# kristi700/ViT-SSL

Hardware: AMD Instinct MI355X
Metric: images_per_sec (higher is better)
Workload: dtype bf16; 1 GPU; ViT-B/16 SimMIM 224x224 mask 0.6 dropout 0.1 AdamW, batch 256/GPU; global_batch=256, parallelism=dp1

## Files before the change

### include/vitssl_hip.h

```cpp
#ifndef VITSSL_HIP_H
#define VITSSL_HIP_H

#include <stdint.h>

#ifdef __cplusplus
extern "C" {
#endif

#define VITSSL_OK 0
#define VITSSL_ERR_ARG (-1)
#define VITSSL_ERR_LAUNCH (-2)

const char* vitssl_last_error(void);
int vitssl_version(void);

int vitssl_set_reserved_cus(int n);
int vitssl_get_reserved_cus(void);
int vitssl_debug_last_nt_grid(void);
int vitssl_debug_last_attn_fwd_grid(void);

typedef struct {
  float p;
  uint32_t site;
  uint64_t seed;
// ... 89 lines not shown
int vitssl_gemm_bf16_tn(const void* A, const void* B, float* C, int64_t M, int N1, int N2, float* workspace,
                        int64_t workspace_floats, void* stream);

typedef struct {
  const void* A;
  const void* B;
  float* C;
  int N1, N2;
} vitssl_tn_job_t;
int64_t vitssl_gemm_tn_batch_workspace_floats(const vitssl_tn_job_t* jobs, int njobs, int64_t M);
int vitssl_gemm_bf16_tn_batch(const vitssl_tn_job_t* jobs, int njobs, int64_t M, float* workspace, int64_t workspace_floats,
                              void* stream);

typedef struct {
  const void* A8;
  const void* B8;
  float* C;
  int N1, N2;
  const float* alpha;
  const float* alpha2;
} vitssl_fp8_tn_job_t;
int64_t vitssl_gemm_fp8_tn_batch_workspace_floats(const vitssl_fp8_tn_job_t* jobs, int njobs, int64_t M);
int vitssl_gemm_fp8_tn_batch(const vitssl_fp8_tn_job_t* jobs, int njobs, int64_t M, float* workspace, int64_t workspace_floats,
                             void* stream);

int vitssl_attn_fwd(const void* qkv, void* out, float* lse, float* probs, int B, int N, int H, int dh,
                    void* stream);
int vitssl_attn_bwd(const void* qkv, const void* out, const void* dout, const float* lse, void* dqkv,
                    float* delta_ws, int B, int N, int H, int dh, void* stream);

int vitssl_patchify_bf16(const float* img, void* patches, int B, int C, int H, int W, int P, void* stream);
int vitssl_gather_patches_f32(const float* img, const int32_t* idx, float* out, int n_idx, int C, int H,
                              int W, int P, void* stream);
int vitssl_gather_rows_bf16(const float* x, const int32_t* idx, void* out, int n_idx, int cols, void* stream);
int vitssl_scatter_rows_f32(const void* src_bf16, const int32_t* inv, float* g, int64_t rows, int cols,
                            void* stream);
int vitssl_gather_cls_f32(const float* x, float* out, int B, int T, int D, void* stream);
int vitssl_scatter_cls_f32(const float* gcls, float* g, int B, int T, int D, void* stream);

int64_t vitssl_embed_bwd_workspace_floats(int B, int tokens, int tok_offset, int D);
int vitssl_embed_bwd(const float* dtok, const uint8_t* mask, void* dproj_bf16, float* dpos, float* dmask_token,
                     float* dbias, float* dcls, int B, int tokens, int tok_offset, int D, float* workspace,
                     int64_t workspace_floats, void* stream);

int vitssl_l1_loss(const float* pred, const float* target, float* loss_sum, void* dpred_bf16, float gscale,
                   int64_t n, float* workspace, int64_t workspace_floats, void* stream);
int vitssl_cross_entropy(const float* logits, const int64_t* labels, float* loss_sum, void* dlogits_bf16,
                         float gscale, int B, int C, void* stream);

int vitssl_colsum_bf16(const void* x_bf16, float* out, int64_t rows, int cols, float* workspace, int64_t workspace_floats,
                       void* stream);

int64_t vitssl_sum_workspace_floats(int64_t rows, int cols);

int vitssl_cast_bf16(const float* src, void* dst, int64_t n, void* stream);
int vitssl_cast_transpose_bf16(const float* src, void* dst, void* dst_t, int R, int C, void* stream);
typedef struct {
  const float* src;
  void* dst;
  void* dst_t;
  int R, C;
} vitssl_cast_job_t;
int vitssl_cast_transpose_batch(const vitssl_cast_job_t* jobs, const int* tile_start, int njobs, int total_tiles,
                                void* stream);
int vitssl_adamw(float* p, const float* g, float* m, float* v, int64_t n, float lr, float beta1, float beta2,
                 float eps, float wd, int step, float gscale, void* stream);
int vitssl_ema(float* teacher, const float* student, int64_t n, float m, void* stream);

int vitssl_rownorm_fwd(const float* z, void* zn_bf16, float* inv_norm, int64_t rows, int cols, void* stream);
int vitssl_rownorm_bwd(const float* dzn, const void* zn_bf16, const float* inv_norm, void* dz_bf16, int64_t rows, int cols,
                       void* stream);
int vitssl_weightnorm_fold(const float* g, const float* v, float* w_f32, float* inv_vnorm, int K, int D, void* stream);
int vitssl_weightnorm_bwd(const float* dw, const float* g, const float* v, const float* inv_vnorm, float* dg, float* dv, int K,
                          int D, void* stream);
#define VITSSL_DINO_TWS_EXTRA(G, B) (8 * (G) * (B))
int64_t vitssl_dino_loss_workspace_floats(int G, int B, int K);
int vitssl_dino_loss(const float* teacher, const float* student, const float* center, float* t_ws, int64_t t_ws_floats,
                     float* loss_sum, void* dstudent_bf16, int G, int V, int B, int K, float teacher_temp, float student_temp,
                     float gscale, void* stream);
int vitssl_colsum_f32(const float* x, float* out, int64_t rows, int cols, void* stream);
int vitssl_center_ema(float* center, const float* colsum, int K, float momentum, float inv_rows, void* stream);

int vitssl_bicubic_resize_fwd(const float* src, float* dst, int gh0, int gw0, int gh, int gw, int D, void* stream);
int vitssl_bicubic_resize_bwd(const float* ddst, float* dsrc, int gh0, int gw0, int gh, int gw, int D, void* stream);

int vitssl_aug_resized_crop_u8(const uint8_t* src, const int32_t* iparams, uint8_t* tmp, uint8_t* dst, int B, int H,
                               int W, int S, void* stream);
int vitssl_aug_color_u8(uint8_t* img, const int32_t* iparams, const float* fparams, int B, int S, void* stream);
int vitssl_aug_blur_to_tensor(const uint8_t* img, const float* fparams, float* out, int B, int S, int ksize,
                              void* stream);

#ifdef __cplusplus
}
#endif
#endif
```

### vit-ssl_amd/csrc/elementwise.hip

```cpp
#include "common.h"

namespace {

constexpr int EW_THREADS = 256;

inline unsigned ew_grid(long long work_items) {
  long long g = (work_items + EW_THREADS - 1) / EW_THREADS;
  if (g < 1) g = 1;
  return (unsigned)g;
}

__global__ void dropout_mask_kernel(unsigned char* keep, long long ngroups, DropKey dk) {
  const long long grp = (long long)blockIdx.x * blockDim.x + threadIdx.x;
  if (grp >= ngroups) return;
  float m[4];
  drop_mult4(dk, (unsigned)grp, m);
  uchar4 o;
  o.x = m[0] != 0.f; o.y = m[1] != 0.f; o.z = m[2] != 0.f; o.w = m[3] != 0.f;
  if (dk.thr == 0) o = make_uchar4(1, 1, 1, 1);
  *(uchar4*)(keep + 4 * grp) = o;
}

template <bool GATHER, typename OutT>
__global__ void patchify_kernel(const float* __restrict__ img, const int* __restrict__ idx, OutT* __restrict__ out,
                                long long nrows, int C, int H, int W, int P) {
  const int gw = W / P, gh = H / P;
  const int pd4 = C * P * P / 4;
  const long long t = (long long)blockIdx.x * blockDim.x + threadIdx.x;
  if (t >= nrows * pd4) return;
  const long long r = t / pd4;
  const int f = (int)(t - r * pd4) * 4;
  const long long m = GATHER ? (long long)idx[r] : r;
  const long long b = m / (gh * gw);
  const int pi = (int)(m - b * gh * gw);
  const int py = pi / gw, px = pi - py * gw;
  const int c = f / (P * P);
  const int kh = (f - c * P * P) / P;
  const int kw = f - c * P * P - kh * P;
  const f32x4 v = *(const f32x4*)(img + ((b * C + c) * H + (py * P + kh)) * (long long)W + px * P + kw);
  if constexpr (sizeof(OutT) == 2) {
    u32x2 w = {pack_bf2(v[0], v[1]), pack_bf2(v[2], v[3])};
    *(u32x2*)((bf16_t*)out + r * (4LL * pd4) + f) = w;
  } else {
    *(f32x4*)((float*)out + r * (4LL * pd4) + f) = v;
  }
}

__global__ void gather_rows_bf16_kernel(const float* __restrict__ x, const int* __restrict__ idx, bf16_t* __restrict__ out,
                                        int n_idx, int cols) {
  const int c4n = cols >> 2;
  const long long t = (long long)blockIdx.x * blockDim.x + threadIdx.x;
  if (t >= (long long)n_idx * c4n) return;
  const int i = (int)(t / c4n);
  const int c = (int)(t - (long long)i * c4n) * 4;
  const f32x4 v = *(const f32x4*)(x + (long long)idx[i] * cols + c);
  u32x2 w = {pack_bf2(v[0], v[1]), pack_bf2(v[2], v[3])};
  *(u32x2*)(out + (long long)i * cols + c) = w;
}

__global__ void scatter_rows_f32_kernel(const bf16_t* __restrict__ src, const int* __restrict__ inv, float* __restrict__ g,
                                        long long rows, int cols) {
  const int c4n = cols >> 2;
  const long long t = (long long)blockIdx.x * blockDim.x + threadIdx.x;
  if (t >= rows * c4n) return;
  const long long r = t / c4n;
  const int c = (int)(t - r * c4n) * 4;
  const int i = inv[r];
  f32x4 v = {0.f, 0.f, 0.f, 0.f};
  if (i >= 0) {
    const u32x2 w = *(const u32x2*)(src + (long long)i * cols + c);
    v = f32x4{bf_lo(w[0]), bf_hi(w[0]), bf_lo(w[1]), bf_hi(w[1])};
  }
  *(f32x4*)(g + r * cols + c) = v;
}

__global__ void gather_cls_kernel(const float* __restrict__ x, float* __restrict__ out, int B, int T, int D) {
  const int d4n = D >> 2;
  const long long t = (long long)blockIdx.x * blockDim.x + threadIdx.x;
  if (t >= (long long)B * d4n) return;
  const int b = (int)(t / d4n);
// ... 160 lines not shown
  __shared__ bf16_t tile[64][66];
  const int b = blockIdx.x;
  int lo = 0, hi = njobs;
  while (hi - lo > 1) {
    const int mid = (lo + hi) >> 1;
    if (tile_start[mid] <= b) lo = mid; else hi = mid;
  }
  const vitssl_cast_job_t j = jobs[lo];
  const int t = b - tile_start[lo];
  const int tx_n = (j.C + 63) >> 6;
  const int r0 = (t / tx_n) * 64, c0 = (t % tx_n) * 64;
  const int R = j.R, C = j.C;
  bf16_t* dst = (bf16_t*)j.dst;
  bf16_t* dst_t = (bf16_t*)j.dst_t;
  const int tx = threadIdx.x & 63, ty = threadIdx.x >> 6;
  for (int rr = ty; rr < 64; rr += 4) {
    const int r = r0 + rr, c = c0 + tx;
    bf16_t h = 0;
    if (r < R && c < C) {
      h = f2bf(j.src[(long long)r * C + c]);
      if (dst) dst[(long long)r * C + c] = h;
    }
    tile[rr][tx] = h;
  }
  __syncthreads();
  if (dst_t) {
    for (int cc = ty; cc < 64; cc += 4) {
      const int c = c0 + cc, r = r0 + tx;
      if (c < C && r < R) dst_t[(long long)c * R + r] = tile[tx][cc];
    }
  }
}

__global__ void adamw_kernel(float* __restrict__ p, const float* __restrict__ g, float* __restrict__ m, float* __restrict__ v,
                             long long n, float lr, float b1, float b2, float eps, float wd, float bc1, float bc2_sqrt,
                             float gscale) {
  const long long n4 = n >> 2;
  const float step_size = lr / bc1;
  for (long long i = (long long)blockIdx.x * blockDim.x + threadIdx.x; i < n4; i += (long long)gridDim.x * blockDim.x) {
    f32x4 pv = *(const f32x4*)(p + 4 * i);
    const f32x4 gv = *(const f32x4*)(g + 4 * i) * gscale;
    f32x4 mv = *(const f32x4*)(m + 4 * i);
    f32x4 vv = *(const f32x4*)(v + 4 * i);
    pv *= (1.f - lr * wd);
    mv = mv * b1 + gv * (1.f - b1);
    vv = vv * b2 + gv * gv * (1.f - b2);
#pragma unroll
    for (int r = 0; r < 4; ++r) pv[r] -= step_size * mv[r] / (sqrtf(vv[r]) / bc2_sqrt + eps);
    *(f32x4*)(p + 4 * i) = pv;
    *(f32x4*)(m + 4 * i) = mv;
    *(f32x4*)(v + 4 * i) = vv;
  }
  if (blockIdx.x == 0 && threadIdx.x < (n & 3)) {
    const long long i = (n4 << 2) + threadIdx.x;
    float pv = p[i] * (1.f - lr * wd);
    const float gv = g[i] * gscale;
    const float mv = m[i] * b1 + gv * (1.f - b1);
    const float vv = v[i] * b2 + gv * gv * (1.f - b2);
    pv -= step_size * mv / (sqrtf(vv) / bc2_sqrt + eps);
    p[i] = pv; m[i] = mv; v[i] = vv;
  }
}

__global__ void ema_kernel(float* __restrict__ t, const float* __restrict__ s, long long n, float mom) {
  const long long n4 = n >> 2;
  const float om = 1.f - mom;
  for (long long i = (long long)blockIdx.x * blockDim.x + threadIdx.x; i < n4; i += (long long)gridDim.x * blockDim.x) {
    const f32x4 tv = *(const f32x4*)(t + 4 * i);
    const f32x4 sv = *(const f32x4*)(s + 4 * i);
    *(f32x4*)(t + 4 * i) = tv * mom + sv * om;
  }
  if (blockIdx.x == 0 && threadIdx.x < (n & 3)) {
    const long long i = (n4 << 2) + threadIdx.x;
    t[i] = t[i] * mom + s[i] * om;
  }
}

__global__ void colsum_bf16_kernel(const bf16_t* __restrict__ x, float* __restrict__ out, long long rows, int cols) {
  const int c = (blockIdx.x * blockDim.x + threadIdx.x) * 4;
  if (c >= cols) return;
  const long long per = (rows + gridDim.y - 1) / gridDim.y;
  const long long r0 = blockIdx.y * per;
  const long long r1 = r0 + per < rows ? r0 + per : rows;
  f32x4 acc = {0.f, 0.f, 0.f, 0.f};
  long long r = r0;
  for (; r + 8 <= r1; r += 8) {
    u32x2 w[8];
#pragma unroll
    for (int u = 0; u < 8; ++u) w[u] = *(const u32x2*)(x + (r + u) * cols + c);
#pragma unroll
    for (int u = 0; u < 8; ++u) acc += f32x4{bf_lo(w[u][0]), bf_hi(w[u][0]), bf_lo(w[u][1]), bf_hi(w[u][1])};
  }
  for (; r < r1; ++r) {
// ... 229 lines not shown
  hipLaunchKernelGGL(cast_bf16_kernel, dim3(stream_grid(n / 4)), dim3(EW_THREADS), 0, (hipStream_t)stream, src, (bf16_t*)dst, (long long)n);
  VS_CHECK_LAUNCH("cast_bf16");
  return VITSSL_OK;
}

extern "C" int vitssl_cast_transpose_bf16(const float* src, void* dst, void* dst_t, int R, int C, void* stream) {
  VS_CHECK_ARG(src && (dst || dst_t) && R > 0 && C > 0, "cast_transpose: bad args");
  hipLaunchKernelGGL(cast_transpose_kernel, dim3((C + 63) / 64, (R + 63) / 64), dim3(EW_THREADS), 0, (hipStream_t)stream, src,
                     (bf16_t*)dst, (bf16_t*)dst_t, R, C);
  VS_CHECK_LAUNCH("cast_transpose");
  return VITSSL_OK;
}

extern "C" int vitssl_cast_transpose_batch(const vitssl_cast_job_t* jobs, const int* tile_start, int njobs, int total_tiles,
                                           void* stream) {
  VS_CHECK_ARG(jobs && tile_start && njobs > 0 && total_tiles > 0, "cast_transpose_batch: bad args");
  hipLaunchKernelGGL(cast_transpose_batch_kernel, dim3(total_tiles), dim3(EW_THREADS), 0, (hipStream_t)stream, jobs, tile_start,
                     njobs);
  VS_CHECK_LAUNCH("cast_transpose_batch");
  return VITSSL_OK;
}

extern "C" int vitssl_adamw(float* p, const float* g, float* m, float* v, int64_t n, float lr, float beta1, float beta2,
                            float eps, float wd, int step, float gscale, void* stream) {
  VS_CHECK_ARG(p && g && m && v && n > 0 && step >= 1, "adamw: bad args");
  const double bc1 = 1.0 - pow((double)beta1, (double)step);
  const double bc2 = 1.0 - pow((double)beta2, (double)step);
  hipLaunchKernelGGL(adamw_kernel, dim3(stream_grid(n / 4)), dim3(EW_THREADS), 0, (hipStream_t)stream, p, g, m, v, (long long)n, lr,
                     beta1, beta2, eps, wd, (float)bc1, (float)sqrt(bc2), gscale);
  VS_CHECK_LAUNCH("adamw");
  return VITSSL_OK;
}

extern "C" int vitssl_ema(float* teacher, const float* student, int64_t n, float m, void* stream) {
  VS_CHECK_ARG(teacher && student && n > 0, "ema: bad args");
  hipLaunchKernelGGL(ema_kernel, dim3(stream_grid(n / 4)), dim3(EW_THREADS), 0, (hipStream_t)stream, teacher, student, (long long)n, m);
  VS_CHECK_LAUNCH("ema");
  return VITSSL_OK;
}
```

### vit-ssl_amd/vit_core/ssl/simmim/model.py

```python
import torch
from torch import nn
from torch.autograd import Function

from ... import _runtime as R
from ..._runtime import BF16, F32, L, ops
from ...encoder_block import EncoderBlock
from .masking import draw_mask, mask_indices_np


class _SimMIMRuntime:

    def __init__(self, model: "SimMIMViT", device):
        self.model = model
        self.device = device
        C, H, W = model.input_shape
        self.P = model.patch_size
        self.C, self.H, self.W = C, H, W
        self.N = (H // self.P) * (W // self.P)
        self.Pd = C * self.P * self.P
        self.D = model.embed_dim
        self.store = R.FlatStore(model, device)
        st = self.store
        prefixes = [f"encoder_blocks.{i}." for i in range(len(model.encoder_blocks))]
        self.stack = R.EncoderStack(st, prefixes, self.D, model.num_heads, model.mlp_dim, model.dropout_p)
        st.register_weight("proj", lambda: st.view("projection.weight", (self.D, self.Pd)), transposed_too=False)
        st.register_weight("head", lambda: st.view("simmim_head.weight", (self.Pd, self.D)))
        self.ws = R.Workspace()
        self.rec = None
        self.save_gen = 0

    def valid_for(self, device) -> bool:
        return device == self.device and self.store.is_attached()

    def embed(self, x, mask_d, tag=""):
        st, ws = self.store, self.ws
        B = x.shape[0]
        M = B * self.N
        patches = ws.get(tag + "patches", (M, self.Pd), BF16, x.device)
        ops.patchify_bf16(x, patches, self.P)
        x0 = ws.get(tag + "x0", (M, self.D), F32, x.device)
        ops.gemm_nt(patches, st.w("proj"), x0, L.EPI_EMBED, bias=st.view("projection.bias"),
                    embed=(mask_d, st.view("mask_token") if mask_d is not None else None,
                           st.view("positional_embedding", (self.N, self.D)), self.N, self.N, 0))
        return x0, patches

    def prepare_mask(self, mask_cpu, dev):
        idx, inv, mflat = mask_indices_np(mask_cpu.contiguous())
        M, Mm = inv.size, idx.size
        key = (M, Mm, str(dev))
        if getattr(self, "_stage_key", None) != key:
            nslots = 4
            self._stage = [dict(idx=torch.empty(Mm, dtype=torch.int32).pin_memory(),
                                inv=torch.empty(M, dtype=torch.int32).pin_memory(),
                                mask=torch.empty(M, dtype=torch.uint8).pin_memory(), ev=None) for _ in range(nslots)]
            self._stage_dev = [dict(idx=torch.empty(Mm, dtype=torch.int32, device=dev),
                                    inv=torch.empty(M, dtype=torch.int32, device=dev),
                                    mask=torch.empty(M, dtype=torch.uint8, device=dev)) for _ in range(nslots)]
            self._stage_pos = 0
            self._stage_key = key
        k = self._stage_pos % len(self._stage)
        self._stage_pos += 1
        slot, d = self._stage[k], self._stage_dev[k]
        if slot["ev"] is not None:
            slot["ev"].synchronize()
        slot["idx"].numpy()[:] = idx
        slot["inv"].numpy()[:] = inv
        slot["mask"].numpy()[:] = mflat
        for name in ("idx", "inv", "mask"):
            d[name].copy_(slot[name], non_blocking=True)
        slot["ev"] = torch.cuda.Event()
        slot["ev"].record(torch.cuda.current_stream())
        return d["idx"], d["inv"], d["mask"]

    def forward(self, x, training: bool, save: bool, mask_cpu=None, prepared=None):
        st, ws = self.store, self.ws
        if x.dim() != 4 or tuple(x.shape[1:]) != (self.C, self.H, self.W):
            raise L.VitsslError(f"SimMIMViT: expected input [B,{self.C},{self.H},{self.W}], got {tuple(x.shape)}")
        self.stack.check_tokens(self.N)
        x = R.as_f32(x)
        B = x.shape[0]
        M = B * self.N
        st.refresh_weights()
        dev = x.device
        if prepared is None:
            if mask_cpu is None:
                mask_cpu = draw_mask(B, self.N, self.model.mask_ratio)
            prepared = self.prepare_mask(mask_cpu, dev)
        seed = R.next_seed() if (training and self.stack.p > 0) else 0
        idx_d, inv_d, mask_d = prepared
        Mm = idx_d.numel()

        targets = torch.empty(Mm, self.Pd, dtype=F32, device=dev)
        if Mm == 0:
            if save:
                self.save_gen += 1
                self.rec = dict(B=B, M=M, Mm=0)
            return torch.empty(0, self.Pd, dtype=F32, device=dev), targets, mask_d.view(B, self.N, 1).bool()
        ops.gather_patches_f32(x, idx_d, targets, self.P)
        tag = "" if save else "tmp."
        x0, patches = self.embed(x, mask_d, tag)
        xL, _ = self.stack.forward(x0, B, self.N, training, seed, save=save, slot="a")
        sel = ws.get(tag + "sel", (Mm, self.D), BF16, dev)
        ops.gather_rows_bf16(xL, idx_d, sel)
        pred = torch.empty(Mm, self.Pd, dtype=F32, device=dev)
        ops.gemm_nt(sel, st.w("head"), pred, L.EPI_F32, bias=st.view("simmim_head.bias"))
        if save:
            self.save_gen += 1
            self.rec = dict(B=B, M=M, Mm=Mm, idx=idx_d, inv=inv_d, mask=mask_d, patches=patches, sel=sel)
        return pred, targets, mask_d.view(B, self.N, 1).bool()

    def backward(self, dpred_bf16, reducer=None):
        st, ws, rec = self.store, self.ws, self.rec
        B, M, Mm = rec["B"], rec["M"], rec["Mm"]
        if Mm == 0:
            if reducer is not None:
                reducer.ready(0, st.gflat.numel())
            return
        dev = dpred_bf16.device
        gv = st.gview
        ops.colsum_bf16(dpred_bf16, gv("simmim_head.bias"))
        ops.gemm_tn(dpred_bf16, rec["sel"], gv("simmim_head.weight", (self.Pd, self.D)))
        dsel = ws.get("dsel", (Mm, self.D), BF16, dev)
        ops.gemm_nt(dpred_bf16, st.w("head.T"), dsel, L.EPI_BF16)
        g = ws.get("g", (M, self.D), F32, dev)
        ops.scatter_rows_f32(dsel, rec["inv"], g)
        if reducer is not None:
            reducer.ready(*st.span("simmim_head.weight", "simmim_head.bias"))
        g = self.stack.backward(g, slot="a", reducer=reducer)
        dproj = ws.get("dproj", (M, self.D), BF16, dev)
        ops.embed_bwd(g, rec["mask"], dproj, gv("positional_embedding", (self.N, self.D)), gv("mask_token"),
                      gv("projection.bias"), None, B, self.N, 0, self.D)
        ops.gemm_tn(dproj, rec["patches"], gv("projection.weight", (self.D, self.Pd)))
        if reducer is not None:
# ... 126 lines not shown
```

### vit-ssl_amd/vitssl_hip/_lib.py

```python
import ctypes as C
import os
import re

_HERE = os.path.dirname(os.path.abspath(__file__))
LIB_PATH = os.environ.get("VITSSL_LIB") or os.path.join(_HERE, "libvitssl_hip.so")
HEADER_PATH = os.path.normpath(os.path.join(_HERE, "..", "..", "include", "vitssl_hip.h"))


class VitsslError(RuntimeError):
    pass


class Dropout(C.Structure):
    _fields_ = [("p", C.c_float), ("site", C.c_uint32), ("seed", C.c_uint64)]


class Embed(C.Structure):
    _fields_ = [("mask", C.c_void_p), ("mask_token", C.c_void_p), ("pos", C.c_void_p),
                ("tokens", C.c_int), ("out_tokens", C.c_int), ("tok_offset", C.c_int)]


class TnJob(C.Structure):
    _fields_ = [("A", C.c_void_p), ("B", C.c_void_p), ("C", C.c_void_p), ("N1", C.c_int), ("N2", C.c_int)]

# ... 14 lines not shown
    _fields_ = [("alpha", C.c_void_p), ("alpha2", C.c_void_p), ("out_fp8", C.c_void_p), ("out_scale", C.c_void_p),
                ("out_amax", C.c_void_p)]


EPI_BF16, EPI_F32, EPI_GELU, EPI_RESID, EPI_DGELU, EPI_EMBED = range(6)

ABI_VERSION = 3
_vp, _i, _i64, _f = C.c_void_p, C.c_int, C.c_int64, C.c_float

PROTOTYPES = {
    "vitssl_dropout_mask": [_vp, _i64, _i64, Dropout, _vp],
    "vitssl_layernorm_fwd": [_vp, _vp, _vp, _vp, _vp, _vp, _i64, _i, _f, _vp],
    "vitssl_layernorm_bwd": [_vp, _vp, _vp, _vp, _vp, _vp, _vp, _vp, _vp, _vp, _vp, Dropout, _i64, _i, _vp, _i64, _vp],
    "vitssl_grad_mask_cast": [_vp, _vp, _vp, Dropout, _i64, _i, _vp, _i64, _vp],
    "vitssl_gemm_bf16_nt": [C.POINTER(Gemm), _vp],
    "vitssl_gemm_bf16_tn": [_vp, _vp, _vp, _i64, _i, _i, _vp, _i64, _vp],
    "vitssl_gemm_bf16_tn_batch": [C.POINTER(TnJob), _i, _i64, _vp, _i64, _vp],
    "vitssl_gemm_fp8_tn_batch": [C.POINTER(Fp8TnJob), _i, _i64, _vp, _i64, _vp],
    "vitssl_gemm_fp8_nt": [C.POINTER(Gemm), C.POINTER(Fp8Gemm), _vp],
    "vitssl_gemm_fp8_tn": [_vp, _vp, _vp, _i64, _i, _i, _vp, _vp, _vp, _i64, _vp],
    "vitssl_quantize_fp8": [_vp, _vp, _i64, _vp],
    "vitssl_attn_bwd_fp8": [_vp, _vp, _vp, _vp, _vp, _vp, _vp, _vp, _i, _i, _i, _i, _vp],
    "vitssl_quantize_fp8_scaled": [_vp, _vp, _i64, _vp, _vp, _vp],
    "vitssl_layernorm_bwd_fp8": [_vp, _vp, _vp, _vp, _vp, _vp, _vp, _vp, _vp, _vp, _vp, _vp, _vp, _vp, Dropout, _i64, _i, _vp, _i64,
                                 _vp],
    "vitssl_grad_mask_cast_fp8": [_vp, _vp, _vp, _vp, _vp, _vp, Dropout, _i64, _i, _vp, _i64, _vp],
    "vitssl_attn_fwd_fp8": [_vp, _vp, _vp, _vp, _vp, _i, _i, _i, _i, _vp],
    "vitssl_layernorm_fwd_fp8": [_vp, _vp, _vp, _vp, _vp, _vp, _vp, _i64, _i, _f, _vp],
    "vitssl_fp8_quantize_weights": [_vp, _vp, _i, _i, _vp, _vp, _vp],
    "vitssl_attn_fwd": [_vp, _vp, _vp, _vp, _i, _i, _i, _i, _vp],
    "vitssl_attn_bwd": [_vp, _vp, _vp, _vp, _vp, _vp, _i, _i, _i, _i, _vp],
    "vitssl_patchify_bf16": [_vp, _vp, _i, _i, _i, _i, _i, _vp],
    "vitssl_gather_patches_f32": [_vp, _vp, _vp, _i, _i, _i, _i, _i, _vp],
    "vitssl_gather_rows_bf16": [_vp, _vp, _vp, _i, _i, _vp],
    "vitssl_scatter_rows_f32": [_vp, _vp, _vp, _i64, _i, _vp],
    "vitssl_gather_cls_f32": [_vp, _vp, _i, _i, _i, _vp],
    "vitssl_scatter_cls_f32": [_vp, _vp, _i, _i, _i, _vp],
    "vitssl_embed_bwd": [_vp, _vp, _vp, _vp, _vp, _vp, _vp, _i, _i, _i, _i, _vp, _i64, _vp],
    "vitssl_l1_loss": [_vp, _vp, _vp, _vp, _f, _i64, _vp, _i64, _vp],
    "vitssl_cross_entropy": [_vp, _vp, _vp, _vp, _f, _i, _i, _vp],
    "vitssl_colsum_bf16": [_vp, _vp, _i64, _i, _vp, _i64, _vp],
    "vitssl_cast_bf16": [_vp, _vp, _i64, _vp],
    "vitssl_cast_transpose_bf16": [_vp, _vp, _vp, _i, _i, _vp],
    "vitssl_cast_transpose_batch": [_vp, _vp, _i, _i, _vp],
    "vitssl_bicubic_resize_fwd": [_vp, _vp, _i, _i, _i, _i, _i, _vp],
    "vitssl_bicubic_resize_bwd": [_vp, _vp, _i, _i, _i, _i, _i, _vp],
    "vitssl_aug_resized_crop_u8": [_vp, _vp, _vp, _vp, _i, _i, _i, _i, _vp],
    "vitssl_aug_color_u8": [_vp, _vp, _vp, _i, _i, _vp],
    "vitssl_aug_blur_to_tensor": [_vp, _vp, _vp, _i, _i, _i, _vp],
    "vitssl_adamw": [_vp, _vp, _vp, _vp, _i64, _f, _f, _f, _f, _f, _i, _f, _vp],
    "vitssl_ema": [_vp, _vp, _i64, _f, _vp],
    "vitssl_rownorm_fwd": [_vp, _vp, _vp, _i64, _i, _vp],
    "vitssl_rownorm_bwd": [_vp, _vp, _vp, _vp, _i64, _i, _vp],
    "vitssl_weightnorm_fold": [_vp, _vp, _vp, _vp, _i, _i, _vp],
    "vitssl_weightnorm_bwd": [_vp, _vp, _vp, _vp, _vp, _vp, _i, _i, _vp],
    "vitssl_dino_loss": [_vp, _vp, _vp, _vp, _i64, _vp, _vp, _i, _i, _i, _i, _f, _f, _f, _vp],
    "vitssl_colsum_f32": [_vp, _vp, _i64, _i, _vp],
    "vitssl_center_ema": [_vp, _vp, _i, _f, _f, _vp],
    "vitssl_set_reserved_cus": [_i],
}

_lib = None


def header_symbols():
    with open(HEADER_PATH) as f:
        txt = f.read()
    return sorted(set(re.findall(r"\b(vitssl_[a-z0-9_]+)\s*\(", txt)))


def lib():
    global _lib
    if _lib is not None:
        return _lib
    if not os.path.exists(LIB_PATH):
        raise VitsslError(
            f"{LIB_PATH} not found: the HIP library is not built. Run `python __graft_entry__.py` "
            "(or __graft_entry__.build()). There is no CPU fallback for the vit_core hot path.")
    import torch
    l = C.CDLL(LIB_PATH)
    l.vitssl_last_error.restype = C.c_char_p
    l.vitssl_last_error.argtypes = []
    l.vitssl_version.restype = C.c_int
# ... 35 lines not shown
```

### vit-ssl_amd/vitssl_hip/engine.py

```python
from __future__ import annotations

from typing import Callable, Dict, List, Optional, Tuple

import torch
from torch import nn

from . import _lib as L
from . import ops

BF16 = torch.bfloat16
F32 = torch.float32
FP8 = ops.FP8
ALIGN = 64
MAX_TOKENS = 2048
FP8_MAX_TOKENS = 256

import os as _os

_LINEAR_OPERANDS = _os.environ.get("VITSSL_LINEAR_OPERANDS", "bf16")


def set_linear_operands(kind: str):
    global _LINEAR_OPERANDS
    if kind not in ("bf16", "fp8"):
# ... 86 lines not shown
    def span(self, first: str, last: str) -> Tuple[int, int]:
        lo = self.offsets[first][0]
        o, n = self.offsets[last]
        return lo, o + n

    def span_view(self, first: str, last: str, shape, grad=False) -> torch.Tensor:
        lo, hi = self.span(first, last)
        buf = self.gflat if grad else self.flat
        v = buf[lo:hi]
        if v.numel() != int(torch.Size(shape).numel()):
            raise L.VitsslError(f"parameters {first}..{last} are not contiguous in the flat store")
        return v.view(shape)

    def attach_grads(self):
        for name, p in zip(self.names, self.params):
            p.grad = self.gview(name, p.shape)

    def mark_dirty(self):
        self.generation += 1

    def weights_key(self):
        pv = 0
        for p in self.params:
            pv += p._version
        return (self.generation, self.flat._version, pv)

    def register_weight(self, key: str, src: Callable[[], torch.Tensor], transposed_too: bool = True, plain: bool = True):
        self._cast_jobs.append((key, src, transposed_too and not self.forward_only, plain))

    def register_fp8_weight(self, key: str, src: Callable[[], torch.Tensor]):
        self._fp8_index[key] = len(self._fp8_jobs)
        self._fp8_jobs.append((key, src))

    def refresh_weights(self):
        key = self.weights_key()
        if key == self._bf16_key and (self._bf16 or self._fp8):
            return
        jobs = []
        for wname, src, tr, plain in self._cast_jobs:
            w = src()
            R, Cn = w.shape
            dst = self._bf16.get(wname) if plain else None
            if plain and (dst is None or dst.shape != (R, Cn)):
                dst = torch.empty(R, Cn, dtype=BF16, device=self.device)
                self._bf16[wname] = dst
            dst_t = None
            if tr:
                dst_t = self._bf16.get(wname + ".T")
                if dst_t is None or dst_t.shape != (Cn, R):
                    dst_t = torch.empty(Cn, R, dtype=BF16, device=self.device)
                    self._bf16[wname + ".T"] = dst_t
            jobs.append((w.contiguous(), dst, dst_t))
        if jobs:
            if getattr(self, "_cast_plan", None) is None:
                self._cast_plan = ops.CastPlan()
            self._cast_plan.run(jobs)
        if self._fp8_jobs:
            jobs8 = []
            for k8, src in self._fp8_jobs:
                w = src()
                R, Cn = w.shape
                dst, dst_t = self._fp8.get(k8), self._fp8.get(k8 + ".T")
                if dst is None or dst.shape != (R, Cn):
                    dst = torch.empty(R, Cn, dtype=FP8, device=self.device)
                    dst_t = torch.empty(Cn, R, dtype=FP8, device=self.device)
                    self._fp8[k8], self._fp8[k8 + ".T"] = dst, dst_t
                jobs8.append((w.contiguous(), dst, dst_t))
            if self._fp8_plan is None:
                self._fp8_plan = ops.Fp8WeightPlan()
            self._fp8_plan.run(jobs8)
        self._bf16_key = key

    def w(self, key: str) -> torch.Tensor:
        return self._bf16[key]

    def w8(self, key: str) -> Tuple[torch.Tensor, torch.Tensor]:
        j = self._fp8_index[key]
        return self._fp8[key], self._fp8_plan.alpha[j:j + 1]

    def w8t(self, key: str) -> Tuple[torch.Tensor, torch.Tensor]:
        j = self._fp8_index[key]
        return self._fp8[key + ".T"], self._fp8_plan.alpha[j:j + 1]


RESERVED_CUS_DEFAULT = 8


def configure_collectives(reserve_cus: int = RESERVED_CUS_DEFAULT):
    if "NCCL_MAX_NCHANNELS" not in _os.environ:
        _os.environ["NCCL_MAX_NCHANNELS"] = str(max(1, int(reserve_cus)))
    if "NCCL_MIN_NCHANNELS" not in _os.environ:
        _os.environ["NCCL_MIN_NCHANNELS"] = str(min(int(_os.environ["NCCL_MAX_NCHANNELS"]), max(1, int(reserve_cus))))
    return {k: _os.environ.get(k) for k in ("NCCL_MAX_NCHANNELS", "NCCL_MIN_NCHANNELS")}


class GradReducer:

    def __init__(self, gflat: torch.Tensor, group=None, bucket_mb: float = 32.0, expect: Optional[Tuple[int, int]] = None,
                 reserve_cus: int = RESERVED_CUS_DEFAULT):
        import torch.distributed as dist
        self.dist = dist
        self.gflat = gflat
        self.group = group
        self.world = dist.get_world_size(group) if dist.is_available() and dist.is_initialized() else 1
# ... 378 lines not shown
```

### vit-ssl_amd/vitssl_hip/ops.py

```python
import ctypes as C

import torch

from . import _lib as L
from ._lib import Dropout, Embed, Fp8Gemm, Gemm, call

BF16 = torch.bfloat16
F32 = torch.float32
FP8 = torch.float8_e4m3fn


def _stream():
    return C.c_void_p(torch.cuda.current_stream().cuda_stream)


def _chk(t, dtype, name, shape=None):
    if t is None:
        raise L.VitsslError(f"{name}: tensor is None")
    if not t.is_cuda:
        raise L.VitsslError(f"{name}: expected a CUDA (HIP) tensor, got {t.device}; there is no CPU fallback")
    if t.device.index != torch.cuda.current_device():
        raise L.VitsslError(f"{name}: tensor lives on {t.device} but the current device is cuda:{torch.cuda.current_device()}; "
                            "call torch.cuda.set_device (one process per GPU) before using the engine")
    if t.dtype != dtype:
# ... 293 lines not shown
         _chk(lse, F32, "lse", (B, H, N)), _opt(probs, F32, "probs", (B, H, N, N)), B, N, H, dh, _stream())


def attn_bwd(qkv, out, dout, lse, dqkv, delta_ws, B, N, H, dh, dqkv_fp8=None, scale=None, amax=None):
    ev = _prof_begin()
    if dqkv_fp8 is not None:
        call("vitssl_attn_bwd_fp8", _chk(qkv, BF16, "qkv", (B * N, 3 * H * dh)), _chk(out, BF16, "out", (B * N, H * dh)),
             _chk(dout, BF16, "dout", (B * N, H * dh)), _chk(lse, F32, "lse", (B, H, N)), _opt(dqkv, BF16, "dqkv", (B * N, 3 * H * dh)),
             _chk(dqkv_fp8, FP8, "dqkv_fp8", (B * N, 3 * H * dh)), _scalar(scale, "scale"), _scalar(amax, "amax"), B, N, H, dh, _stream())
    else:
        _attn_bwd(qkv, out, dout, lse, dqkv, delta_ws, B, N, H, dh)
    _prof_end(ev, f"attn_bwd B{B} N{N} H{H}", 8.0 * B * H * N * N * dh)


def _attn_bwd(qkv, out, dout, lse, dqkv, delta_ws, B, N, H, dh):
    call("vitssl_attn_bwd", _chk(qkv, BF16, "qkv", (B * N, 3 * H * dh)), _chk(out, BF16, "out", (B * N, H * dh)),
         _chk(dout, BF16, "dout", (B * N, H * dh)), _chk(lse, F32, "lse", (B, H, N)),
         _chk(dqkv, BF16, "dqkv", (B * N, 3 * H * dh)), _chk(delta_ws, F32, "delta_ws", (B, H, N)), B, N, H, dh, _stream())


def patchify_bf16(img, patches, P):
    B, Cc, H, W = img.shape
    call("vitssl_patchify_bf16", _chk(img, F32, "img"), _chk(patches, BF16, "patches", (B * (H // P) * (W // P), Cc * P * P)),
         B, Cc, H, W, P, _stream())


def gather_patches_f32(img, idx, out, P):
    B, Cc, H, W = img.shape
    n = idx.numel()
    call("vitssl_gather_patches_f32", _chk(img, F32, "img"), _chk(idx, torch.int32, "idx"), _chk(out, F32, "out", (n, Cc * P * P)),
         n, Cc, H, W, P, _stream())


def gather_rows_bf16(x, idx, out):
    rows, cols = x.shape
    n = idx.numel()
    call("vitssl_gather_rows_bf16", _chk(x, F32, "x"), _chk(idx, torch.int32, "idx"), _chk(out, BF16, "out", (n, cols)), n, cols, _stream())


def scatter_rows_f32(src, inv, g):
    rows, cols = g.shape
    call("vitssl_scatter_rows_f32", _chk(src, BF16, "src"), _chk(inv, torch.int32, "inv", (rows,)), _chk(g, F32, "g"), rows, cols, _stream())


def gather_cls_f32(x, out, B, T, D):
    call("vitssl_gather_cls_f32", _chk(x, F32, "x", (B * T, D)), _chk(out, F32, "out", (B, D)), B, T, D, _stream())


def scatter_cls_f32(gcls, g, B, T, D):
    call("vitssl_scatter_cls_f32", _chk(gcls, F32, "gcls", (B, D)), _chk(g, F32, "g", (B * T, D)), B, T, D, _stream())


def embed_bwd(dtok, mask, dproj, dpos, dmask_token, dbias, dcls, B, tokens, tok_offset, D):
    T_out = tokens + tok_offset
    wsn = int(L.lib().vitssl_embed_bwd_workspace_floats(B, tokens, tok_offset, D))
    ws = _tn_workspace(dtok.device, wsn)
    call("vitssl_embed_bwd", _chk(dtok, F32, "dtok", (B * T_out, D)), _opt(mask, torch.uint8, "mask", (B * tokens,)),
         _chk(dproj, BF16, "dproj", (B * tokens, D)), _opt(dpos, F32, "dpos", (T_out, D)),
         _opt(dmask_token, F32, "dmask_token", (D,)), _opt(dbias, F32, "dbias", (D,)), _opt(dcls, F32, "dcls", (D,)),
         B, tokens, tok_offset, D, C.c_void_p(ws.data_ptr()), ws.numel(), _stream())


def l1_loss(pred, target, loss_sum, dpred=None, gscale=0.0):
    n = pred.numel()
    call("vitssl_l1_loss", _chk(pred, F32, "pred"), _chk(target, F32, "target", pred.shape), _chk(loss_sum, F32, "loss_sum", (1,)),
         _opt(dpred, BF16, "dpred", pred.shape), float(gscale), n, *_sum_ws(pred.device, n, 1), _stream())


def cross_entropy(logits, labels, loss_sum, dlogits=None, gscale=0.0):
    B, Cn = logits.shape
    call("vitssl_cross_entropy", _chk(logits, F32, "logits"), _chk(labels, torch.int64, "labels", (B,)),
         _chk(loss_sum, F32, "loss_sum", (1,)), _opt(dlogits, BF16, "dlogits", (B, Cn)), float(gscale), B, Cn, _stream())


def colsum_bf16(x, out):
    rows, cols = x.shape
    call("vitssl_colsum_bf16", _chk(x, BF16, "x"), _chk(out, F32, "out", (cols,)), rows, cols, *_sum_ws(x.device, rows, cols), _stream())


def cast_bf16(src, dst):
    call("vitssl_cast_bf16", _chk(src, F32, "src"), _chk(dst, BF16, "dst", src.shape), src.numel(), _stream())


def cast_transpose_bf16(src, dst, dst_t):
    R, Cn = src.shape
    call("vitssl_cast_transpose_bf16", _chk(src, F32, "src"), _opt(dst, BF16, "dst", (R, Cn)), _opt(dst_t, BF16, "dst_t", (Cn, R)),
         R, Cn, _stream())


class CastPlan:

    def __init__(self):
        self.key = None
        self.jobs_dev = None
        self.starts_dev = None
        self.njobs = 0
        self.total = 0
        self.keep = None

    def run(self, jobs):
        import numpy as np
        key = tuple((s.data_ptr(), 0 if d is None else d.data_ptr(), 0 if t is None else t.data_ptr(), s.shape[0], s.shape[1])
                    for s, d, t in jobs)
        if key != self.key:
            for s, d, t in jobs:
                R, Cn = s.shape
                _chk(s, F32, "src"); _opt(d, BF16, "dst", (R, Cn)); _opt(t, BF16, "dst_t", (Cn, R))
            dev = jobs[0][0].device
            rec = np.zeros(len(jobs), dtype=np.dtype([("src", "<u8"), ("dst", "<u8"), ("dst_t", "<u8"), ("R", "<i4"), ("C", "<i4")]))
            starts = np.zeros(len(jobs) + 1, dtype=np.int32)
            for i, k in enumerate(key):
                rec[i] = k
                starts[i + 1] = starts[i] + ((k[3] + 63) // 64) * ((k[4] + 63) // 64)
            self.jobs_dev = torch.from_numpy(rec.view(np.uint8).copy()).to(dev)
            self.starts_dev = torch.from_numpy(starts).to(dev)
            self.njobs, self.total, self.key = len(jobs), int(starts[-1]), key
        self.keep = jobs
        call("vitssl_cast_transpose_batch", C.c_void_p(self.jobs_dev.data_ptr()), C.c_void_p(self.starts_dev.data_ptr()),
             self.njobs, self.total, _stream())


class Fp8WeightPlan:

    def __init__(self):
        self.key = None
        self.jobs_dev = self.starts_dev = self.amax = self.alpha = None
        self.njobs = self.total = 0
        self.keep = None

    def run(self, jobs):
        import numpy as np
        key = tuple((s.data_ptr(), 0 if d is None else d.data_ptr(), 0 if t is None else t.data_ptr(), s.shape[0], s.shape[1])
                    for s, d, t in jobs)
        if key != self.key:
            for s, d, t in jobs:
                R, Cn = s.shape
                _chk(s, F32, "src"); _opt(d, FP8, "dst", (R, Cn)); _opt(t, FP8, "dst_t", (Cn, R))
            dev = jobs[0][0].device
            rec = np.zeros(len(jobs), dtype=np.dtype([("src", "<u8"), ("dst", "<u8"), ("dst_t", "<u8"), ("R", "<i4"), ("C", "<i4")]))
            starts = np.zeros(len(jobs) + 1, dtype=np.int32)
            for i, k in enumerate(key):
                rec[i] = k
                starts[i + 1] = starts[i] + ((k[3] + 63) // 64) * ((k[4] + 63) // 64)
            self.jobs_dev = torch.from_numpy(rec.view(np.uint8).copy()).to(dev)
            self.starts_dev = torch.from_numpy(starts).to(dev)
            self.amax = torch.zeros(len(jobs), dtype=F32, device=dev)
            self.alpha = torch.ones(len(jobs), dtype=F32, device=dev)
            self.njobs, self.total, self.key = len(jobs), int(starts[-1]), key
        self.keep = jobs
        call("vitssl_fp8_quantize_weights", C.c_void_p(self.jobs_dev.data_ptr()), C.c_void_p(self.starts_dev.data_ptr()),
             self.njobs, self.total, C.c_void_p(self.amax.data_ptr()), C.c_void_p(self.alpha.data_ptr()), _stream())

# ... 101 lines not shown
```

### vit-ssl_amd/vitssl_hip/optim.py

```python
import torch

from . import ops
from .engine import FlatStore


class FusedAdamW(torch.optim.Optimizer):

    def __init__(self, store: FlatStore, lr=1e-3, betas=(0.9, 0.999), eps=1e-8, weight_decay=1e-2):
        params = [p for p in store.params if p.requires_grad]
        defaults = dict(lr=lr, betas=betas, eps=eps, weight_decay=weight_decay)
        super().__init__(params, defaults)
        self.store = store
        self.exp_avg = torch.zeros_like(store.flat)
        self.exp_avg_sq = torch.zeros_like(store.flat)
        self.step_count = 0
        self._all_trainable = len(params) == len(store.params)

    def _hyper(self):
        g = self.param_groups[0]
        return float(g["lr"]), g["betas"][0], g["betas"][1], g["eps"], g["weight_decay"]

    @torch.no_grad()
    def step_flat(self, gscale: float = 1.0):
        if not self._all_trainable:
            return self.step(gscale=gscale, from_flat=True)
        lr, b1, b2, eps, wd = self._hyper()
        self.step_count += 1
        st = self.store
        ops.adamw(st.flat, st.gflat, self.exp_avg, self.exp_avg_sq, lr, b1, b2, eps, wd, self.step_count, gscale)
        st.mark_dirty()

    @torch.no_grad()
    def step(self, closure=None, gscale: float = 1.0, from_flat: bool = False):
        loss = None
        if closure is not None:
            with torch.enable_grad():
                loss = closure()
        lr, b1, b2, eps, wd = self._hyper()
        self.step_count += 1
        st = self.store
        trainable = {id(p) for p in self.param_groups[0]["params"]}
        for name, p in zip(st.names, st.params):
            if id(p) not in trainable or (p.grad is None and not from_flat):
                continue
            o, n = st.offsets[name]
            gslice = st.gflat[o:o + n]
            if not from_flat and p.grad.data_ptr() != gslice.data_ptr():
                gslice.copy_(p.grad.reshape(-1))
            ops.adamw(st.flat[o:o + n], gslice, self.exp_avg[o:o + n], self.exp_avg_sq[o:o + n], lr, b1, b2, eps, wd,
                      self.step_count, gscale)
        st.mark_dirty()
        return loss

    def state_dict(self):
        st = self.store
        state = {}
        trainable = [p for p in self.param_groups[0]["params"]]
        index = {id(p): i for i, p in enumerate(trainable)}
        for name, p in zip(st.names, st.params):
            if id(p) not in index:
                continue
            o, n = st.offsets[name]
            state[index[id(p)]] = {
# ... 25 lines not shown
```

Measured before the change: 7875 images/s.

## Fuse AdamW with bf16 weight cast/transpose and patchify with target gather

Adds a fused kernel that runs the AdamW update and writes the bf16 weight copies and their transposes from the freshly updated fp32 values in the same pass. Parameters not covered by the cast table are updated by extra blocks that look up their spans with a binary search. This removes the separate pass that re-read the fp32 weights to refresh the bf16 images. A second fused kernel patchifies the image to bf16 and writes the fp32 targets for masked patches in one read, replacing the separate gather. The cost is more complex kernel and plan bookkeeping, plus a fallback path when alignment conditions fail or fp8 jobs exist.

```diff
diff --git a/include/vitssl_hip.h b/include/vitssl_hip.h
--- a/include/vitssl_hip.h
+++ b/include/vitssl_hip.h
@@ -145,6 +145,8 @@
 int vitssl_patchify_bf16(const float* img, void* patches, int B, int C, int H, int W, int P, void* stream);
 int vitssl_gather_patches_f32(const float* img, const int32_t* idx, float* out, int n_idx, int C, int H,
                               int W, int P, void* stream);
+int vitssl_patchify_targets(const float* img, const int32_t* inv, void* patches, float* targets, int B, int C, int H,
+                            int W, int P, void* stream);
 int vitssl_gather_rows_bf16(const float* x, const int32_t* idx, void* out, int n_idx, int cols, void* stream);
 int vitssl_scatter_rows_f32(const void* src_bf16, const int32_t* inv, float* g, int64_t rows, int cols,
                             void* stream);
@@ -178,6 +180,9 @@
                                 void* stream);
 int vitssl_adamw(float* p, const float* g, float* m, float* v, int64_t n, float lr, float beta1, float beta2,
                  float eps, float wd, int step, float gscale, void* stream);
+int vitssl_adamw_cast(float* p, const float* g, float* m, float* v, int64_t n, const vitssl_cast_job_t* jobs,
+                      const int* tile_start, int njobs, int total_tiles, const int64_t* rest, int nrest, int64_t rest_quads,
+                      float lr, float beta1, float beta2, float eps, float wd, int step, float gscale, void* stream);
 int vitssl_ema(float* teacher, const float* student, int64_t n, float m, void* stream);
 
 int vitssl_rownorm_fwd(const float* z, void* zn_bf16, float* inv_norm, int64_t rows, int cols, void* stream);
diff --git a/vit-ssl_amd/csrc/elementwise.hip b/vit-ssl_amd/csrc/elementwise.hip
--- a/vit-ssl_amd/csrc/elementwise.hip
+++ b/vit-ssl_amd/csrc/elementwise.hip
@@ -46,6 +46,27 @@
   }
 }
 
+__global__ void patchify_targets_kernel(const float* __restrict__ img, const int* __restrict__ inv, bf16_t* __restrict__ out,
+                                        float* __restrict__ tgt, long long nrows, int C, int H, int W, int P) {
+  const int gw = W / P, gh = H / P;
+  const int pd4 = C * P * P / 4;
+  const long long t = (long long)blockIdx.x * blockDim.x + threadIdx.x;
+  if (t >= nrows * pd4) return;
+  const long long r = t / pd4;
+  const int f = (int)(t - r * pd4) * 4;
+  const long long b = r / (gh * gw);
+  const int pi = (int)(r - b * gh * gw);
+  const int py = pi / gw, px = pi - py * gw;
+  const int c = f / (P * P);
+  const int kh = (f - c * P * P) / P;
+  const int kw = f - c * P * P - kh * P;
+  const f32x4 v = *(const f32x4*)(img + ((b * C + c) * H + (py * P + kh)) * (long long)W + px * P + kw);
+  u32x2 w = {pack_bf2(v[0], v[1]), pack_bf2(v[2], v[3])};
+  *(u32x2*)(out + r * (4LL * pd4) + f) = w;
+  const int i = inv[r];
+  if (i >= 0) *(f32x4*)(tgt + (long long)i * (4LL * pd4) + f) = v;
+}
+
 __global__ void gather_rows_bf16_kernel(const float* __restrict__ x, const int* __restrict__ idx, bf16_t* __restrict__ out,
                                         int n_idx, int cols) {
   const int c4n = cols >> 2;
@@ -272,25 +293,35 @@
   }
 }
 
+struct AdamwHyper {
+  float lr, b1, b2, eps, wd, step_size, bc2_sqrt, gscale;
+};
+
+__device__ __forceinline__ f32x4 adamw_quad(float* __restrict__ p, const float* __restrict__ g, float* __restrict__ m,
+                                            float* __restrict__ v, long long e, const AdamwHyper& h) {
+  f32x4 pv = *(const f32x4*)(p + e);
+  const f32x4 gv = *(const f32x4*)(g + e) * h.gscale;
+  f32x4 mv = *(const f32x4*)(m + e);
+  f32x4 vv = *(const f32x4*)(v + e);
+  pv *= (1.f - h.lr * h.wd);
+  mv = mv * h.b1 + gv * (1.f - h.b1);
+  vv = vv * h.b2 + gv * gv * (1.f - h.b2);
+#pragma unroll
+  for (int r = 0; r < 4; ++r) pv[r] -= h.step_size * mv[r] / (sqrtf(vv[r]) / h.bc2_sqrt + h.eps);
+  *(f32x4*)(p + e) = pv;
+  *(f32x4*)(m + e) = mv;
+  *(f32x4*)(v + e) = vv;
+  return pv;
+}
+
 __global__ void adamw_kernel(float* __restrict__ p, const float* __restrict__ g, float* __restrict__ m, float* __restrict__ v,
                              long long n, float lr, float b1, float b2, float eps, float wd, float bc1, float bc2_sqrt,
                              float gscale) {
   const long long n4 = n >> 2;
   const float step_size = lr / bc1;
-  for (long long i = (long long)blockIdx.x * blockDim.x + threadIdx.x; i < n4; i += (long long)gridDim.x * blockDim.x) {
-    f32x4 pv = *(const f32x4*)(p + 4 * i);
-    const f32x4 gv = *(const f32x4*)(g + 4 * i) * gscale;
-    f32x4 mv = *(const f32x4*)(m + 4 * i);
-    f32x4 vv = *(const f32x4*)(v + 4 * i);
-    pv *= (1.f - lr * wd);
-    mv = mv * b1 + gv * (1.f - b1);
-    vv = vv * b2 + gv * gv * (1.f - b2);
-#pragma unroll
-    for (int r = 0; r < 4; ++r) pv[r] -= step_size * mv[r] / (sqrtf(vv[r]) / bc2_sqrt + eps);
-    *(f32x4*)(p + 4 * i) = pv;
-    *(f32x4*)(m + 4 * i) = mv;
-    *(f32x4*)(v + 4 * i) = vv;
-  }
+  const AdamwHyper h = {lr, b1, b2, eps, wd, step_size, bc2_sqrt, gscale};
+  for (long long i = (long long)blockIdx.x * blockDim.x + threadIdx.x; i < n4; i += (long long)gridDim.x * blockDim.x)
+    adamw_quad(p, g, m, v, 4 * i, h);
   if (blockIdx.x == 0 && threadIdx.x < (n & 3)) {
     const long long i = (n4 << 2) + threadIdx.x;
     float pv = p[i] * (1.f - lr * wd);
@@ -299,6 +330,67 @@
     const float vv = v[i] * b2 + gv * gv * (1.f - b2);
     pv -= step_size * mv / (sqrtf(vv) / bc2_sqrt + eps);
     p[i] = pv; m[i] = mv; v[i] = vv;
+  }
+}
+
+constexpr int AC_LD = 68;
+__global__ __launch_bounds__(EW_THREADS) void adamw_cast_kernel(float* __restrict__ p, const float* __restrict__ g,
+                                                                float* __restrict__ m, float* __restrict__ v,
+                                                                const vitssl_cast_job_t* __restrict__ jobs,
+                                                                const int* __restrict__ tile_start, int njobs, int total_tiles,
+                                                                const long long* __restrict__ rest, int nrest, AdamwHyper h, float bc1) {
+  h.step_size = h.lr / bc1;
+  const int b = blockIdx.x;
+  if (b >= total_tiles) {
+    const long long* qs = rest + nrest;
+    const long long nq = qs[nrest];
+    const long long stride = (long long)(gridDim.x - total_tiles) * blockDim.x;
+    for (long long q = (long long)(b - total_tiles) * blockDim.x + threadIdx.x; q < nq; q += stride) {
+      int lo = 0, hi = nrest;
+      while (hi - lo > 1) {
+        const int mid = (lo + hi) >> 1;
+        if (qs[mid] <= q) lo = mid; else hi = mid;
+      }
+      adamw_quad(p, g, m, v, rest[lo] + 4 * (q - qs[lo]), h);
+    }
+    return;
+  }
+  __shared__ __attribute__((aligned(16))) bf16_t tile[64][AC_LD];
+  int lo = 0, hi = njobs;
+  while (hi - lo > 1) {
+    const int mid = (lo + hi) >> 1;
+    if (tile_start[mid] <= b) lo = mid; else hi = mid;
+  }
+  const vitssl_cast_job_t j = jobs[lo];
+  const int t = b - tile_start[lo];
+  const int tx_n = (j.C + 63) >> 6;
+  const int r0 = (t / tx_n) * 64, c0 = (t % tx_n) * 64;
+  const int R = j.R, C = j.C;
+  const long long base = j.src - p;
+  bf16_t* dst = (bf16_t*)j.dst;
+  bf16_t* dst_t = (bf16_t*)j.dst_t;
+  const int tx = (threadIdx.x & 15) * 4, ty = threadIdx.x >> 4;
+#pragma unroll
+  for (int rr = ty; rr < 64; rr += 16) {
+    const int r = r0 + rr, c = c0 + tx;
+    u32x2 w = {0u, 0u};
+    if (r < R && c < C) {
+      const f32x4 pv = adamw_quad(p, g, m, v, base + (long long)r * C + c, h);
+      w = u32x2{pack_bf2(pv[0], pv[1]), pack_bf2(pv[2], pv[3])};
+      if (dst) *(u32x2*)(dst + (long long)r * C + c) = w;
+    }
+    *(u32x2*)&tile[rr][tx] = w;
+  }
+  if (!dst_t) return;
+  __syncthreads();
+#pragma unroll
+  for (int cc = ty; cc < 64; cc += 16) {
+    const int c = c0 + cc, r = r0 + tx;
+    if (c < C && r < R) {
+      const u32x2 w = {(unsigned)tile[tx][cc] | ((unsigned)tile[tx + 1][cc] << 16),
+                       (unsigned)tile[tx + 2][cc] | ((unsigned)tile[tx + 3][cc] << 16)};
+      *(u32x2*)(dst_t + (long long)c * R + r) = w;
+    }
   }
 }
 
@@ -594,6 +686,36 @@
   return VITSSL_OK;
 }
 
+extern "C" int vitssl_adamw_cast(float* p, const float* g, float* m, float* v, int64_t n, const vitssl_cast_job_t* jobs,
+                                 const int* tile_start, int njobs, int total_tiles, const int64_t* rest, int nrest, int64_t rest_quads,
+                                 float lr, float beta1, float beta2, float eps, float wd, int step, float gscale, void* stream) {
+  VS_CHECK_ARG(p && g && m && v && n > 0 && n % 4 == 0 && step >= 1, "adamw_cast: bad args (n=%lld must be a multiple of 4)", (long long)n);
+  VS_CHECK_ARG(jobs && tile_start && njobs > 0 && total_tiles > 0, "adamw_cast: empty cast table");
+  VS_CHECK_ARG(rest_quads >= 0 && (rest_quads == 0 || (rest && nrest > 0)), "adamw_cast: bad rest table");
+  VS_CHECK_ARG(((uintptr_t)p | (uintptr_t)g | (uintptr_t)m | (uintptr_t)v) % 16 == 0, "adamw_cast: buffers must be 16-byte aligned");
+  const double bc1 = 1.0 - pow((double)beta1, (double)step);
+  const double bc2 = 1.0 - pow((double)beta2, (double)step);
+  const AdamwHyper h = {lr, beta1, beta2, eps, wd, 0.f, (float)sqrt(bc2), gscale};
+  long long rb = (rest_quads + EW_THREADS - 1) / EW_THREADS;
+  if (rb > 1024) rb = 1024;
+  hipLaunchKernelGGL(adamw_cast_kernel, dim3((unsigned)(total_tiles + rb)), dim3(EW_THREADS), 0, (hipStream_t)stream, p, g, m, v, jobs,
+                     tile_start, njobs, total_tiles, (const long long*)rest, nrest, h, (float)bc1);
+  VS_CHECK_LAUNCH("adamw_cast");
+  return VITSSL_OK;
+}
+
+extern "C" int vitssl_patchify_targets(const float* img, const int32_t* inv, void* patches, float* targets, int B, int C, int H, int W,
+                                       int P, void* stream) {
+  VS_CHECK_ARG(img && inv && patches && targets, "patchify_targets: null pointer");
+  if (int rc = check_patch_args("patchify_targets", B, C, H, W, P)) return rc;
+  const long long nrows = (long long)B * (H / P) * (W / P);
+  const long long work = nrows * (C * P * P / 4);
+  hipLaunchKernelGGL(patchify_targets_kernel, dim3(ew_grid(work)), dim3(EW_THREADS), 0, (hipStream_t)stream, img, inv, (bf16_t*)patches,
+                     targets, nrows, C, H, W, P);
+  VS_CHECK_LAUNCH("patchify_targets");
+  return VITSSL_OK;
+}
+
 extern "C" int vitssl_ema(float* teacher, const float* student, int64_t n, float m, void* stream) {
   VS_CHECK_ARG(teacher && student && n > 0, "ema: bad args");
   hipLaunchKernelGGL(ema_kernel, dim3(stream_grid(n / 4)), dim3(EW_THREADS), 0, (hipStream_t)stream, teacher, student, (long long)n, m);
diff --git a/vit-ssl_amd/vit_core/ssl/simmim/model.py b/vit-ssl_amd/vit_core/ssl/simmim/model.py
--- a/vit-ssl_amd/vit_core/ssl/simmim/model.py
+++ b/vit-ssl_amd/vit_core/ssl/simmim/model.py
@@ -32,12 +32,13 @@
     def valid_for(self, device) -> bool:
         return device == self.device and self.store.is_attached()
 
-    def embed(self, x, mask_d, tag=""):
+    def embed(self, x, mask_d, tag="", patches=None):
         st, ws = self.store, self.ws
         B = x.shape[0]
         M = B * self.N
-        patches = ws.get(tag + "patches", (M, self.Pd), BF16, x.device)
-        ops.patchify_bf16(x, patches, self.P)
+        if patches is None:
+            patches = ws.get(tag + "patches", (M, self.Pd), BF16, x.device)
+            ops.patchify_bf16(x, patches, self.P)
         x0 = ws.get(tag + "x0", (M, self.D), F32, x.device)
         ops.gemm_nt(patches, st.w("proj"), x0, L.EPI_EMBED, bias=st.view("projection.bias"),
                     embed=(mask_d, st.view("mask_token") if mask_d is not None else None,
@@ -96,9 +97,10 @@
                 self.save_gen += 1
                 self.rec = dict(B=B, M=M, Mm=0)
             return torch.empty(0, self.Pd, dtype=F32, device=dev), targets, mask_d.view(B, self.N, 1).bool()
-        ops.gather_patches_f32(x, idx_d, targets, self.P)
         tag = "" if save else "tmp."
-        x0, patches = self.embed(x, mask_d, tag)
+        patches = ws.get(tag + "patches", (M, self.Pd), BF16, dev)
+        ops.patchify_targets(x, inv_d, patches, targets, self.P)
+        x0, patches = self.embed(x, mask_d, tag, patches)
         xL, _ = self.stack.forward(x0, B, self.N, training, seed, save=save, slot="a")
         sel = ws.get(tag + "sel", (Mm, self.D), BF16, dev)
         ops.gather_rows_bf16(xL, idx_d, sel)
diff --git a/vit-ssl_amd/vitssl_hip/_lib.py b/vit-ssl_amd/vitssl_hip/_lib.py
--- a/vit-ssl_amd/vitssl_hip/_lib.py
+++ b/vit-ssl_amd/vitssl_hip/_lib.py
@@ -70,6 +70,7 @@
     "vitssl_attn_bwd": [_vp, _vp, _vp, _vp, _vp, _vp, _i, _i, _i, _i, _vp],
     "vitssl_patchify_bf16": [_vp, _vp, _i, _i, _i, _i, _i, _vp],
     "vitssl_gather_patches_f32": [_vp, _vp, _vp, _i, _i, _i, _i, _i, _vp],
+    "vitssl_patchify_targets": [_vp, _vp, _vp, _vp, _i, _i, _i, _i, _i, _vp],
     "vitssl_gather_rows_bf16": [_vp, _vp, _vp, _i, _i, _vp],
     "vitssl_scatter_rows_f32": [_vp, _vp, _vp, _i64, _i, _vp],
     "vitssl_gather_cls_f32": [_vp, _vp, _i, _i, _i, _vp],
@@ -87,6 +88,7 @@
     "vitssl_aug_color_u8": [_vp, _vp, _vp, _i, _i, _vp],
     "vitssl_aug_blur_to_tensor": [_vp, _vp, _vp, _i, _i, _i, _vp],
     "vitssl_adamw": [_vp, _vp, _vp, _vp, _i64, _f, _f, _f, _f, _f, _i, _f, _vp],
+    "vitssl_adamw_cast": [_vp, _vp, _vp, _vp, _i64, _vp, _vp, _i, _i, _vp, _i, _i64, _f, _f, _f, _f, _f, _i, _f, _vp],
     "vitssl_ema": [_vp, _vp, _i64, _f, _vp],
     "vitssl_rownorm_fwd": [_vp, _vp, _vp, _i64, _i, _vp],
     "vitssl_rownorm_bwd": [_vp, _vp, _vp, _vp, _i64, _i, _vp],
diff --git a/vit-ssl_amd/vitssl_hip/engine.py b/vit-ssl_amd/vitssl_hip/engine.py
--- a/vit-ssl_amd/vitssl_hip/engine.py
+++ b/vit-ssl_amd/vitssl_hip/engine.py
@@ -142,10 +142,7 @@
         self._fp8_index[key] = len(self._fp8_jobs)
         self._fp8_jobs.append((key, src))
 
-    def refresh_weights(self):
-        key = self.weights_key()
-        if key == self._bf16_key and (self._bf16 or self._fp8):
-            return
+    def _bf16_jobs(self):
         jobs = []
         for wname, src, tr, plain in self._cast_jobs:
             w = src()
@@ -161,10 +158,20 @@
                     dst_t = torch.empty(Cn, R, dtype=BF16, device=self.device)
                     self._bf16[wname + ".T"] = dst_t
             jobs.append((w.contiguous(), dst, dst_t))
+        return jobs
+
+    def _plan(self):
+        if getattr(self, "_cast_plan", None) is None:
+            self._cast_plan = ops.CastPlan()
+        return self._cast_plan
+
+    def refresh_weights(self):
+        key = self.weights_key()
+        if key == self._bf16_key and (self._bf16 or self._fp8):
+            return
+        jobs = self._bf16_jobs()
         if jobs:
-            if getattr(self, "_cast_plan", None) is None:
-                self._cast_plan = ops.CastPlan()
-            self._cast_plan.run(jobs)
+            self._plan().run(jobs)
         if self._fp8_jobs:
             jobs8 = []
             for k8, src in self._fp8_jobs:
@@ -180,6 +187,16 @@
                 self._fp8_plan = ops.Fp8WeightPlan()
             self._fp8_plan.run(jobs8)
         self._bf16_key = key
+
+    def adamw_with_images(self, exp_avg, exp_avg_sq, lr, beta1, beta2, eps, wd, step, gscale) -> bool:
+        if not self._cast_jobs or self._fp8_jobs:
+            return False
+        if not self._plan().run_adamw(self._bf16_jobs(), self.flat, self.gflat, exp_avg, exp_avg_sq, lr, beta1, beta2, eps, wd, step,
+                                      gscale):
+            return False
+        self.generation += 1
+        self._bf16_key = self.weights_key()
+        return True
 
     def w(self, key: str) -> torch.Tensor:
         return self._bf16[key]
diff --git a/vit-ssl_amd/vitssl_hip/ops.py b/vit-ssl_amd/vitssl_hip/ops.py
--- a/vit-ssl_amd/vitssl_hip/ops.py
+++ b/vit-ssl_amd/vitssl_hip/ops.py
@@ -349,6 +349,15 @@
          n, Cc, H, W, P, _stream())
 
 
+def patchify_targets(img, inv, patches, targets, P):
+    B, Cc, H, W = img.shape
+    rows = B * (H // P) * (W // P)
+    if targets.dim() != 2 or targets.shape[1] != Cc * P * P:
+        raise L.VitsslError(f"targets: expected [n_masked, {Cc * P * P}], got {tuple(targets.shape)}")
+    call("vitssl_patchify_targets", _chk(img, F32, "img"), _chk(inv, torch.int32, "inv", (rows,)),
+         _chk(patches, BF16, "patches", (rows, Cc * P * P)), _chk(targets, F32, "targets"), B, Cc, H, W, P, _stream())
+
+
 def gather_rows_bf16(x, idx, out):
     rows, cols = x.shape
     n = idx.numel()
@@ -414,8 +423,9 @@
         self.njobs = 0
         self.total = 0
         self.keep = None
-
-    def run(self, jobs):
+        self.rest_key = None
+
+    def _upload(self, jobs):
         import numpy as np
         key = tuple((s.data_ptr(), 0 if d is None else d.data_ptr(), 0 if t is None else t.data_ptr(), s.shape[0], s.shape[1])
                     for s, d, t in jobs)
@@ -432,9 +442,54 @@
             self.jobs_dev = torch.from_numpy(rec.view(np.uint8).copy()).to(dev)
             self.starts_dev = torch.from_numpy(starts).to(dev)
             self.njobs, self.total, self.key = len(jobs), int(starts[-1]), key
+            self.rest_key = None
+
+    def run(self, jobs):
+        self._upload(jobs)
         self.keep = jobs
         call("vitssl_cast_transpose_batch", C.c_void_p(self.jobs_dev.data_ptr()), C.c_void_p(self.starts_dev.data_ptr()),
              self.njobs, self.total, _stream())
+
+    def run_adamw(self, jobs, p, g, m, v, lr, beta1, beta2, eps, wd, step, gscale=1.0):
+        import numpy as np
+        self._upload(jobs)
+        n = p.numel()
+        rkey = (p.data_ptr(), n)
+        if rkey != self.rest_key:
+            _chk(p, F32, "p")
+            self.rest_key, self.rest_ok = rkey, False
+            spans = []
+            for s, _, _ in jobs:
+                off, rem = divmod(s.data_ptr() - p.data_ptr(), 4)
+                R, Cn = s.shape
+                if rem or off % 4 or R % 4 or Cn % 4 or off < 0 or off + R * Cn > n:
+                    return False
+                spans.append((off, off + R * Cn))
+            spans.sort()
+            begins, quads, pos = [], [0], 0
+            for lo, hi in spans + [(n, n)]:
+                if lo < pos:
+                    return False
+                if lo > pos:
+                    begins.append(pos)
+                    quads.append(quads[-1] + (lo - pos) // 4)
+                pos = hi
+            if n % 4:
+                return False
+            self.nrest, self.rest_quads = len(begins), quads[-1]
+            self.rest_dev = torch.from_numpy(np.array(begins + quads, dtype=np.int64)).to(p.device)
+            self.rest_ok = True
+        if not self.rest_ok:
+            return False
+        self.keep = jobs
+        ev = _prof_begin()
+        call("vitssl_adamw_cast", _chk(p, F32, "p"), _chk(g, F32, "g", p.shape), _chk(m, F32, "m", p.shape), _chk(v, F32, "v", p.shape),
+             n, C.c_void_p(self.jobs_dev.data_ptr()), C.c_void_p(self.starts_dev.data_ptr()), self.njobs, self.total,
+             C.c_void_p(self.rest_dev.data_ptr() if self.nrest else 0), self.nrest, self.rest_quads, float(lr), float(beta1),
+             float(beta2), float(eps), float(wd), int(step), float(gscale), _stream())
+        nimg = sum((0 if d is None else d.numel()) + (0 if t is None else t.numel()) for _, d, t in jobs)
+        _prof_end(ev, "adamw", 0.0, 28 * n + 2 * nimg)
+        return True
 
 
 class Fp8WeightPlan:
diff --git a/vit-ssl_amd/vitssl_hip/optim.py b/vit-ssl_amd/vitssl_hip/optim.py
--- a/vit-ssl_amd/vitssl_hip/optim.py
+++ b/vit-ssl_amd/vitssl_hip/optim.py
@@ -27,8 +27,9 @@
         lr, b1, b2, eps, wd = self._hyper()
         self.step_count += 1
         st = self.store
-        ops.adamw(st.flat, st.gflat, self.exp_avg, self.exp_avg_sq, lr, b1, b2, eps, wd, self.step_count, gscale)
-        st.mark_dirty()
+        if not st.adamw_with_images(self.exp_avg, self.exp_avg_sq, lr, b1, b2, eps, wd, self.step_count, gscale):
+            ops.adamw(st.flat, st.gflat, self.exp_avg, self.exp_avg_sq, lr, b1, b2, eps, wd, self.step_count, gscale)
+            st.mark_dirty()
 
     @torch.no_grad()
     def step(self, closure=None, gscale: float = 1.0, from_flat: bool = False):
```

After: 7923 images/s (median of 6 runs). No clear change (+0.6%).
